# VITA-Group/UVC

Measured on AMD Instinct MI355X. Metric: images/sec UVC Stage-1 step, DeiT-Tiny budget=0.5, higher is better.
Workload: dtype bf16; 1 GPU; deit_tiny_patch16_224 Stage-1 UVC-train step, budget 0.5, per-GPU batch 512, 224x224x3 synthetic, soft distillation alpha 0.1, block gating on; global_batch=512, parallelism=dp1

## Files before the change

uvc_amd/csrc/fused_mlp.hip:

```cpp
#include "common.h"
#include "../../include/uvc_kernels.h"
#include <utility>
#include <algorithm>

namespace {

typedef bf16_t T;
constexpr int D = 192, KT = 6, RW = 2;
constexpr int W1S = D * 2 + 32;

__device__ __forceinline__ f32x4 mma(const bf16x8& a, const bf16x8& b, f32x4 c) {
  return __builtin_amdgcn_mfma_f32_16x16x32_bf16(a, b, c, 0, 0, 0);
}
__device__ __forceinline__ u32x4 pack8u(const f32x4& lo, const f32x4& hi) {
  u32x4 r;
  r[0] = pack_bf16x2(lo[0], lo[1]); r[1] = pack_bf16x2(lo[2], lo[3]);
  r[2] = pack_bf16x2(hi[0], hi[1]); r[3] = pack_bf16x2(hi[2], hi[3]);
  return r;
}
__device__ __forceinline__ bf16x8 pack8(const f32x4& lo, const f32x4& hi) { return __builtin_bit_cast(bf16x8, pack8u(lo, hi)); }

constexpr int V3_NW = 4, V3_NTH = 64 * V3_NW, V3_ROWS = V3_NW * RW * 16, V3_FC = 32;
constexpr int V3_W2S = V3_FC * 2 + 32;
constexpr int V3_W1B = V3_FC * W1S, V3_W2B = D * V3_W2S;
// ... 170 lines not shown
  f32x4 acc[RW][2], gpv[RW][2];
  auto fc1 = [&](int c) {
    const unsigned w1a = w1lane + (unsigned)((c & 1) * V3_BUF);
    const unsigned ba = b1lane + (unsigned)(c * (V3_FC * 4));
    u32x4 bi[2], f1[3][2];
    bi[0] = ds_rd<0>(ba); bi[1] = ds_rd<16>(ba);
    f1[0][0] = ds_rd<0>(w1a); f1[0][1] = ds_rd<16 * W1S>(w1a);
    f1[1][0] = ds_rd<64>(w1a); f1[1][1] = ds_rd<16 * W1S + 64>(w1a);
    __builtin_amdgcn_sched_barrier(0);
    static_for<KT>([&](auto ksv) {
      constexpr int ks = ksv.value, cur = ks % 3, nxt = (ks + 2) % 3;
      wait_tie2<(ks + 1 < KT) ? 2 : 0>(f1[cur][0], f1[cur][1]);
      if constexpr (ks == 0) asm volatile("" : "+v"(bi[0]), "+v"(bi[1]));
      static_for<2>([&](auto tv) {
        constexpr int t = tv.value;
        const bf16x8 af = __builtin_bit_cast(bf16x8, f1[cur][t]);
#pragma unroll
        for (int r = 0; r < RW; ++r) acc[r][t] = mma(af, hf[r][ks], ks == 0 ? __builtin_bit_cast(f32x4, bi[t]) : acc[r][t]);
        if constexpr (ks + 2 < KT) f1[nxt][t] = ds_rd<t * 16 * W1S + (ks + 2 < KT ? ks + 2 : 0) * 64>(w1a);
        __builtin_amdgcn_sched_barrier(0);
      });
    });
  };
  auto fc2_gelu = [&](auto fc2v, auto geluv, int cprev) {
    constexpr bool FC2 = decltype(fc2v)::value, GELU = decltype(geluv)::value;
    const unsigned w2a = w2lane + (unsigned)((cprev & 1) * V3_BUF);
    u32x4 f2[6];
    if constexpr (FC2) {
      static_for<6>([&](auto jv) { f2[jv.value] = ds_rd<jv.value * 16 * V3_W2S>(w2a); });
      __builtin_amdgcn_sched_barrier(0);
    }
    static_for<12>([&](auto jv) {
      constexpr int j = jv.value, slot = j % 6;
      if constexpr (FC2) {
        constexpr int younger = (j < 6) ? 5 : 11 - j;
        asm volatile("s_waitcnt lgkmcnt(%1)" : "+v"(f2[slot]) : "n"(younger));
        const bf16x8 af = __builtin_bit_cast(bf16x8, f2[slot]);
#pragma unroll
        for (int r = 0; r < RW; ++r) out[r][j] = mma(af, uf[r], out[r][j]);
        if constexpr (j + 6 < 12) f2[slot] = ds_rd<(j + 6 < 12 ? j + 6 : 0) * 16 * V3_W2S>(w2a);
      }
      if constexpr (GELU && j < 8) {
        constexpr int r = j >> 2, t = (j >> 1) & 1, e0 = (j & 1) * 2;
        if constexpr (TRAIN) {
          float f0, g0, f1, g1;
          Gelu<T>::fg(acc[r][t][e0], f0, g0);
          Gelu<T>::fg(acc[r][t][e0 + 1], f1, g1);
          acc[r][t][e0] = f0; gpv[r][t][e0] = g0; acc[r][t][e0 + 1] = f1; gpv[r][t][e0 + 1] = g1;
        } else {
          acc[r][t][e0] = Gelu<T>::f(acc[r][t][e0]);
          acc[r][t][e0 + 1] = Gelu<T>::f(acc[r][t][e0 + 1]);
        }
      }
      __builtin_amdgcn_sched_barrier(0);
    });
    if constexpr (GELU) {
#pragma unroll
      for (int r = 0; r < RW; ++r) {
        uf[r] = pack8(acc[r][0], acc[r][1]);
        if constexpr (TRAIN) {
          const int row = m0 + r * 16 + li;
          if (row < a.M) {
            const size_t o = (size_t)row * a.F + (size_t)(cprev + 1) * V3_FC + g * 8;
            *reinterpret_cast<u32x4*>(reinterpret_cast<T*>(a.u) + o) = __builtin_bit_cast(u32x4, uf[r]);
            *reinterpret_cast<u32x4*>(reinterpret_cast<T*>(a.gp) + o) = pack8u(gpv[r][0], gpv[r][1]);
          }
        }
      }
    }
  };
  auto end_iter = [&]() {
    asm volatile("s_waitcnt vmcnt(0)" ::: "memory");
    __builtin_amdgcn_s_barrier();
    __builtin_amdgcn_sched_barrier(0);
  };
  {
    dma(1, 0);
    __builtin_amdgcn_sched_barrier(0);
    fc1(0);
    fc2_gelu(std::false_type{}, std::true_type{}, -1);
    end_iter();
  }
  for (int c = 1; c < nch; ++c) {
    dma(c + 1, c);
    __builtin_amdgcn_sched_barrier(0);
    fc1(c);
    fc2_gelu(std::true_type{}, std::true_type{}, c - 1);
    end_iter();
  }
  fc2_gelu(std::true_type{}, std::false_type{}, nch - 1);

#pragma unroll
  for (int r = 0; r < RW; ++r) {
    const int row = m0 + r * 16 + li;
    if (row < a.M) {
      char* orow = reinterpret_cast<char*>(a.out) + (size_t)row * D * RSZ;
#pragma unroll
      for (int j = 0; j < D / 16; ++j) {
        const int col = j * 16 + g * 4;
        f32x4 o = out[r][j];
        if (a.gate) {
          f32x4 xp;
          if constexpr (RLOW) {
            const u32x2 q = *reinterpret_cast<const u32x2*>(reinterpret_cast<const bf16_t*>(a.x_prev) + (size_t)row * D + col);
            xp = f32x4{__uint_as_float(q[0] << 16), __uint_as_float(q[0] & 0xffff0000u), __uint_as_float(q[1] << 16), __uint_as_float(q[1] & 0xffff0000u)};
          } else xp = *reinterpret_cast<const f32x4*>(reinterpret_cast<const float*>(a.x_prev) + (size_t)row * D + col);
#pragma unroll
          for (int e = 0; e < 4; ++e) o[e] = __builtin_fmaf(d1, o[e], __builtin_fmaf(d0, xp[e], 0.0f));
        }
        if constexpr (RLOW) {
          u32x2 q; q[0] = pack_bf16x2(o[0], o[1]); q[1] = pack_bf16x2(o[2], o[3]);
          *reinterpret_cast<u32x2*>(orow + col * 2) = q;
          o = f32x4{__uint_as_float(q[0] << 16), __uint_as_float(q[0] & 0xffff0000u), __uint_as_float(q[1] << 16), __uint_as_float(q[1] & 0xffff0000u)};
        } else *reinterpret_cast<f32x4*>(orow + col * 4) = o;
        out[r][j] = o;
      }
    }
  }
  if (a.next_h) {
#pragma unroll
    for (int r = 0; r < RW; ++r) {
      const int row = m0 + r * 16 + li;
      float s = 0.f;
#pragma unroll
      for (int j = 0; j < D / 16; ++j) s += (out[r][j][0] + out[r][j][1]) + (out[r][j][2] + out[r][j][3]);
      s = sum_rows4(s);
      const float mean = s * (1.0f / D);
      float q = 0.f;
#pragma unroll
      for (int j = 0; j < D / 16; ++j)
#pragma unroll
        for (int e = 0; e < 4; ++e) { const float dd = out[r][j][e] - mean; q += dd * dd; }
      q = sum_rows4(q);
      const float rstd = rsqrtf(q * (1.0f / D) + a.eps);
      if (row < a.M) {
        if (a.next_mean && g == 0) { a.next_mean[row] = mean; a.next_rstd[row] = rstd; }
        T* hrow = reinterpret_cast<T*>(a.next_h) + (size_t)row * D;
#pragma unroll
        for (int j = 0; j < D / 16; ++j) {
          const int col = j * 16 + g * 4;
          const f32x4 gm = *reinterpret_cast<const f32x4*>(a.next_gamma + col), bt = *reinterpret_cast<const f32x4*>(a.next_beta + col);
          float y[4];
#pragma unroll
          for (int e = 0; e < 4; ++e) y[e] = (out[r][j][e] - mean) * rstd * gm[e] + bt[e];
          u32x2 pk; pk[0] = pack_bf16x2(y[0], y[1]); pk[1] = pack_bf16x2(y[2], y[3]);
          *reinterpret_cast<u32x2*>(hrow + col) = pk;
        }
      }
    }
  }
  asm volatile("s_waitcnt vmcnt(0)" ::: "memory");
}

constexpr int P_NW = 8, P_NTH = 64 * P_NW, P_MIN_ROWS = 16384, P_PASS = 13;
constexpr int P_W1B = V3_FC * D * 2, P_W2B = D * V3_FC * 2;
constexpr int P_BUF = P_W1B + P_W2B, P_NBUF = 3;
constexpr int P_XT = 16 * D * 2;
constexpr int P_OFF_X = P_NBUF * P_BUF;
constexpr int P_OFF_B1 = P_OFF_X + P_PASS * P_XT;
constexpr int P_OFF_GB = P_OFF_B1 + 4096, P_LDS = P_OFF_GB + 5 * D * 4;
constexpr int P_ND = (P_BUF / 1024 - P_NW / 2) / (P_NW / 2);
constexpr int P_NR = P_XT / 1024;
static_assert(P_LDS <= 160 * 1024, "one workgroup per CU");
static_assert(P_XT % 1024 == 0 && P_BUF == (P_ND + 1) * (P_NW / 2) * 1024 && P_PASS <= 13, "whole DMA instructions; four loader waves, four slots each");
static_assert(P_NW * P_XT + 256 < 65536, "second-tile offsets are ds_read immediates");

template <int OFF> __device__ __forceinline__ u32x2 ds_rd64(unsigned addr) {
  u32x2 v;
  asm volatile("ds_read_b64 %0, %1 offset:%2" : "=v"(v) : "v"(addr), "n"(OFF));
  return v;
}
__device__ __forceinline__ f32x4 bf4(const u32x2& q) {
  return f32x4{__uint_as_float(q[0] << 16), __uint_as_float(q[0] & 0xffff0000u), __uint_as_float(q[1] << 16), __uint_as_float(q[1] & 0xffff0000u)};
}
template <int N> __device__ __forceinline__ void wait_vm() { asm volatile("s_waitcnt vmcnt(%0)" ::"n"(N) : "memory"); }

__global__ __launch_bounds__(P_NTH, 1) void k_mlp_fused_p(uvc_mlp_args a, int ntiles) {
  extern __shared__ __attribute__((aligned(16))) char smem[];
  const int tid = threadIdx.x, lane = tid & 63, g = lane >> 4, li = lane & 15;
  const int w = __builtin_amdgcn_readfirstlane(tid >> 6);
  const int nch = a.F / V3_FC;
  {
    float* const sB1 = reinterpret_cast<float*>(smem + P_OFF_B1);
    float* const sG = reinterpret_cast<float*>(smem + P_OFF_GB);
    for (int i = tid; i < a.F; i += P_NTH) sB1[i] = a.b1[i];
    if (tid < D) {
      sG[tid] = a.gamma[tid]; sG[D + tid] = a.beta[tid]; sG[2 * D + tid] = a.b2[tid];
      if (a.next_h) { sG[3 * D + tid] = a.next_gamma[tid]; sG[4 * D + tid] = a.next_beta[tid]; }
    }
  }
  float d0 = 0.f, d1 = 1.f;
  if (a.gate) { d0 = a.gate[0]; d1 = a.gate[1]; }
  const unsigned s0 = lds_addr(smem);
  const int t0 = (int)((long long)blockIdx.x * ntiles / gridDim.x), t1 = (int)((long long)(blockIdx.x + 1) * ntiles / gridDim.x);
  int npass = (t1 - t0 + P_PASS - 1) / P_PASS;
  auto tile_rows = [&](int pb, int cnt, int k) { return (k < cnt) ? (pb + k) * 16 : a.M; };

  auto rowdma = [&](int npb, int ncnt, int q) {
    int ln = lane;
    asm volatile("" : "+v"(ln));
    const char* xb = reinterpret_cast<const char*>(a.x);
    const int slot = (q < 3 || w == P_NW / 2) ? (w & 3) + 4 * q : (w & 3) + 8;
    const int mb = tile_rows(npb, ncnt, slot);
#pragma unroll
    for (int i = 0; i < P_XT / 1024; ++i) {
      const int n = i * 64 + ln, row = n / 24, sp = n - row * 24;
      int grow = mb + row;
      grow = grow < a.M ? grow : a.M - 1;
      const unsigned off = (unsigned)grow * (unsigned)(D * 2) + (unsigned)((sp ^ ((row >> 1) & 7)) * 16);
      __builtin_amdgcn_global_load_lds((const void __attribute__((address_space(1)))*)(xb + (unsigned long long)off),
                                       (void __attribute__((address_space(3)))*)(smem + P_OFF_X + slot * P_XT + i * 1024), 16, 0, 0);
    }
  };

  unsigned doff[P_ND];
  const char* gsrc[P_ND];
  unsigned gstep[P_ND], ldst[P_ND];
  bool isw1[P_ND];
#pragma unroll
  for (int q = 0; q < P_ND; ++q) {
    const int j = (w < P_NW / 2) ? w : w + 4 * q;
    if (j < P_W1B / 1024) {
      const int n = j * 64 + lane, lr = n / 24, sp = n - lr * 24;
      const int h = ((lr >> 2) & 3) * 8 + (lr >> 4) * 4 + (lr & 3);
      doff[q] = (unsigned)(h * D * 2 + (sp ^ ((lr >> 1) & 7)) * 16);
      gsrc[q] = reinterpret_cast<const char*>(a.w1); gstep[q] = (unsigned)(V3_FC * D * 2);
      ldst[q] = (unsigned)(j * 1024);
    } else {
      const int jj = j - P_W1B / 1024;
      const int n = jj * 64 + lane, row = n >> 2, sp = n & 3;
      doff[q] = (unsigned)(row * a.F * 2 + (sp ^ ((4 - (row >> 2)) & 3)) * 16);
      gsrc[q] = reinterpret_cast<const char*>(a.w2); gstep[q] = (unsigned)(V3_FC * 2);
      ldst[q] = (unsigned)(P_W1B + jj * 1024);
    }
    isw1[q] = j < P_W1B / 1024;
  }
  auto dma = [&](auto nv, int c1, unsigned o1, int c2, unsigned o2) {
#pragma unroll
    for (int q = 0; q < decltype(nv)::value; ++q) {
      const int cc = isw1[q] ? c1 : c2;
      const char* src = gsrc[q] + (unsigned long long)((unsigned)cc * gstep[q] + doff[q]);
      char* dst = smem + ldst[q] + (isw1[q] ? o1 : o2);
      __builtin_amdgcn_global_load_lds((const void __attribute__((address_space(1)))*)src, (void __attribute__((address_space(3)))*)dst, 16, 0, 0);
    }
  };

  const int fx = (li >> 1) & 7;
  const unsigned sw0 = (unsigned)(li * (D * 2) + (g ^ fx) * 16), sw1 = (unsigned)(li * (D * 2) + ((4 + g) ^ fx) * 16);
  const unsigned xe0 = s0 + (unsigned)(P_OFF_X + w * P_XT) + sw0, xe1 = s0 + (unsigned)(P_OFF_X + w * P_XT) + sw1;
  unsigned xo[4];
#pragma unroll
  for (int q = 0; q < 4; ++q) xo[q] = s0 + (unsigned)(P_OFF_X + w * P_XT + li * (D * 2) + (((2 * q + (g >> 1)) ^ fx) * 16) + (g & 1) * 8);
  const unsigned w1e0 = s0 + sw0, w1e1 = s0 + sw1;
  const unsigned w2lane = s0 + (unsigned)(P_W1B + li * (V3_FC * 2) + ((g ^ ((4 - (li >> 2)) & 3)) * 16));
  const unsigned b1lane = s0 + (unsigned)(P_OFF_B1 + g * 32);
  const unsigned ga = s0 + (unsigned)(P_OFF_GB + g * 32), ba = ga + (unsigned)(D * 4);
  const unsigned b2a = s0 + (unsigned)(P_OFF_GB + 2 * D * 4 + g * 16), nga = b2a + (unsigned)(D * 4), nba = nga + (unsigned)(D * 4);

  unsigned o_cur = 0, o_nxt = P_BUF, o_nn = 2 * P_BUF;
  int pb = t0, cnt = (t1 - t0 + npass - 1) / (npass > 0 ? npass : 1);
  int mb0 = tile_rows(pb, cnt, w), mb1 = tile_rows(pb, cnt, P_NW + w);
  const bool loader = w >= P_NW / 2;
  if (loader) {
#pragma unroll
    for (int q = 0; q < 4; ++q) rowdma(pb, cnt, q);
    dma(std::integral_constant<int, P_ND>{}, 0, o_cur, 0, o_cur);
    dma(std::integral_constant<int, P_ND>{}, 1, o_nxt, 0, o_cur);
  } else {
    dma(std::integral_constant<int, 1>{}, 0, o_cur, 0, o_cur);
    dma(std::integral_constant<int, 1>{}, 1, o_nxt, 0, o_cur);
  }
  wait_vm<0>();
  __syncthreads();
  __builtin_amdgcn_sched_barrier(0);

  bf16x8 hf[RW][KT];
  f32x4 out[RW][D / 16];
  bf16x8 uf[RW];
  f32x4 acc[RW][2];

  auto pass = [&](auto ntv, auto ldv, int npb, int ncnt) {
    constexpr int NT = decltype(ntv)::value;
    constexpr bool LD = decltype(ldv)::value;
    static_for<NT>([&](auto rv) {
      constexpr int r = rv.value, XR = r * P_NW * P_XT;
      const int mb = r ? mb1 : mb0;
      u32x4 xq[KT];
      static_for<KT>([&](auto ksv) { constexpr int ks = ksv.value; xq[ks] = ds_rd<XR + (ks >> 1) * 128>((ks & 1) ? xe1 : xe0); });
      asm volatile("s_waitcnt lgkmcnt(0)" : "+v"(xq[0]), "+v"(xq[1]), "+v"(xq[2]), "+v"(xq[3]), "+v"(xq[4]), "+v"(xq[5]));
      f32x4 xv[2 * KT];
#pragma unroll
      for (int ks = 0; ks < KT; ++ks) {
        const u32x4 q = xq[ks];
        xv[2 * ks] = f32x4{__uint_as_float(q[0] << 16), __uint_as_float(q[0] & 0xffff0000u), __uint_as_float(q[1] << 16), __uint_as_float(q[1] & 0xffff0000u)};
        xv[2 * ks + 1] = f32x4{__uint_as_float(q[2] << 16), __uint_as_float(q[2] & 0xffff0000u), __uint_as_float(q[3] << 16), __uint_as_float(q[3] & 0xffff0000u)};
      }
      const float okf = (mb + li) < a.M ? 1.0f : 0.0f;
      float s = 0.f;
#pragma unroll
      for (int i = 0; i < 2 * KT; ++i) s += (xv[i][0] + xv[i][1]) + (xv[i][2] + xv[i][3]);
      s = sum_rows4(s);
      const float mean = s * (1.0f / D);
      float q = 0.f;
#pragma unroll
      for (int i = 0; i < 2 * KT; ++i)
#pragma unroll
        for (int e = 0; e < 4; ++e) { const float d = xv[i][e] - mean; q += d * d; }
      q = sum_rows4(q);
      const float rstd = rsqrtf(q * (1.0f / D) + a.eps);
      __builtin_amdgcn_sched_barrier(0);
      static_for<KT>([&](auto ksv) {
        constexpr int ks = ksv.value;
        u32x4 gq0 = ds_rd<ks * 128>(ga), gq1 = ds_rd<ks * 128 + 16>(ga), bq0 = ds_rd<ks * 128>(ba), bq1 = ds_rd<ks * 128 + 16>(ba);
        asm volatile("s_waitcnt lgkmcnt(0)" : "+v"(gq0), "+v"(gq1), "+v"(bq0), "+v"(bq1));
        const f32x4 g0 = __builtin_bit_cast(f32x4, gq0), g1 = __builtin_bit_cast(f32x4, gq1);
        const f32x4 b0 = __builtin_bit_cast(f32x4, bq0), b1 = __builtin_bit_cast(f32x4, bq1);
        f32x4 y0, y1;
#pragma unroll
        for (int e = 0; e < 4; ++e) {
          y0[e] = ((xv[2 * ks][e] - mean) * rstd * g0[e] + b0[e]) * okf;
          y1[e] = ((xv[2 * ks + 1][e] - mean) * rstd * g1[e] + b1[e]) * okf;
        }
        hf[r][ks] = pack8(y0, y1);
        asm volatile("" : "+v"(hf[r][ks]));
        __builtin_amdgcn_sched_barrier(0);
      });
      static_for<D / 64>([&](auto jqv) {
        constexpr int j0 = jqv.value * 4;
        u32x2 xr[4];
        u32x4 bq[4];
        static_for<4>([&](auto qv) {
          constexpr int j = j0 + qv.value;
          xr[qv.value] = ds_rd64<XR + (j >> 2) * 128>(xo[j & 3]);
          bq[qv.value] = ds_rd<j * 64>(b2a);
        });
        asm volatile("s_waitcnt lgkmcnt(0)" : "+v"(xr[0]), "+v"(xr[1]), "+v"(xr[2]), "+v"(xr[3]), "+v"(bq[0]), "+v"(bq[1]), "+v"(bq[2]), "+v"(bq[3]));
#pragma unroll
        for (int q4 = 0; q4 < 4; ++q4) {
          const f32x4 x4 = bf4(xr[q4]), bv = __builtin_bit_cast(f32x4, bq[q4]);
#pragma unroll
          for (int e = 0; e < 4; ++e) out[r][j0 + q4][e] = x4[e] + bv[e];
          asm volatile("" : "+v"(out[r][j0 + q4]));
        }
        __builtin_amdgcn_sched_barrier(0);
      });
    });
    __builtin_amdgcn_sched_barrier(0);

    auto fc1 = [&](int c) {
      const unsigned a0 = w1e0 + o_cur, a1 = w1e1 + o_cur;
      const unsigned bia = b1lane + (unsigned)(c * (V3_FC * 4));
      u32x4 bi[2], f1[3][2];
      bi[0] = ds_rd<0>(bia); bi[1] = ds_rd<16>(bia);
      f1[0][0] = ds_rd<0>(a0); f1[0][1] = ds_rd<16 * D * 2>(a0);
      f1[1][0] = ds_rd<0>(a1); f1[1][1] = ds_rd<16 * D * 2>(a1);
      __builtin_amdgcn_sched_barrier(0);
      static_for<KT>([&](auto ksv) {
        constexpr int ks = ksv.value, cur = ks % 3, nxt = (ks + 2) % 3;
        wait_tie2<(ks + 1 < KT) ? 2 : 0>(f1[cur][0], f1[cur][1]);
        if constexpr (ks == 0) asm volatile("" : "+v"(bi[0]), "+v"(bi[1]));
        static_for<2>([&](auto tv) {
          constexpr int t = tv.value;
          const bf16x8 af = __builtin_bit_cast(bf16x8, f1[cur][t]);
#pragma unroll
          for (int r = 0; r < NT; ++r) acc[r][t] = mma(af, hf[r][ks], ks == 0 ? __builtin_bit_cast(f32x4, bi[t]) : acc[r][t]);
          if constexpr (ks + 2 < KT) f1[nxt][t] = ds_rd<t * 16 * D * 2 + ((ks + 2 < KT ? ks + 2 : 0) >> 1) * 128>((ks & 1) ? a1 : a0);
          __builtin_amdgcn_sched_barrier(0);
        });
      });
    };
    auto fc2_gelu = [&](auto fc2v, auto geluv) {
      constexpr bool FC2 = decltype(fc2v)::value, GELU = decltype(geluv)::value;
      const unsigned w2a = w2lane + o_nn;
      u32x4 f2[6];
      if constexpr (FC2) {
        static_for<6>([&](auto jv) { f2[jv.value] = ds_rd<jv.value * 1024>(w2a); });
        __builtin_amdgcn_sched_barrier(0);
      }
      static_for<12>([&](auto jv) {
        constexpr int j = jv.value, slot = j % 6;
        if constexpr (FC2) {
          constexpr int younger = (j < 6) ? 5 : 11 - j;
          asm volatile("s_waitcnt lgkmcnt(%1)" : "+v"(f2[slot]) : "n"(younger));
          const bf16x8 af = __builtin_bit_cast(bf16x8, f2[slot]);
#pragma unroll
          for (int r = 0; r < NT; ++r) out[r][j] = mma(af, uf[r], out[r][j]);
          if constexpr (j + 6 < 12) f2[slot] = ds_rd<(j + 6 < 12 ? j + 6 : 0) * 1024>(w2a);
        }
        if constexpr (GELU && j < 8) {
          if constexpr (NT == 2) {
            constexpr int r = j >> 2, t = (j >> 1) & 1, e0 = (j & 1) * 2;
            acc[r][t][e0] = Gelu<T>::f(acc[r][t][e0]);
            acc[r][t][e0 + 1] = Gelu<T>::f(acc[r][t][e0 + 1]);
          } else {
            constexpr int t = j >> 2, e = j & 3;
            acc[0][t][e] = Gelu<T>::f(acc[0][t][e]);
          }
        }
        __builtin_amdgcn_sched_barrier(0);
      });
      if constexpr (GELU) {
#pragma unroll
        for (int r = 0; r < NT; ++r) uf[r] = pack8(acc[r][0], acc[r][1]);
      }
    };
    auto rotate = [&]() { const unsigned t = o_cur; o_cur = o_nxt; o_nxt = o_nn; o_nn = t; };
    auto request = [&](int c) {
      const int c1 = c + 2 < nch ? c + 2 : c + 2 - nch, c2 = c + 1 < nch ? c + 1 : 0;
      dma(std::integral_constant<int, LD ? P_ND : 1>{}, c1, o_nn, c2, o_nxt);
    };
    __builtin_amdgcn_s_barrier();
    __builtin_amdgcn_sched_barrier(0);
    {
      request(0);
      if constexpr (LD) rowdma(npb, ncnt, 0);
      __builtin_amdgcn_sched_barrier(0);
      fc1(0);
      fc2_gelu(std::false_type{}, std::true_type{});
      wait_vm<LD ? P_ND + P_NR : 1>();
      __builtin_amdgcn_s_barrier();
      __builtin_amdgcn_sched_barrier(0);
      rotate();
    }
#pragma nounroll
    for (int c = 1; c < 4; ++c) {
      request(c);
      if constexpr (LD) rowdma(npb, ncnt, c);
      __builtin_amdgcn_sched_barrier(0);
      fc1(c);
      fc2_gelu(std::true_type{}, std::true_type{});
      wait_vm<LD ? P_ND + 2 * P_NR : 1>();
      __builtin_amdgcn_s_barrier();
      __builtin_amdgcn_sched_barrier(0);
      rotate();
    }
#pragma nounroll
    for (int c = 4; c < nch; ++c) {
      request(c);
      __builtin_amdgcn_sched_barrier(0);
      fc1(c);
      fc2_gelu(std::true_type{}, std::true_type{});
      if (LD && c == 4) wait_vm<LD ? P_ND + P_NR : 1>(); else wait_vm<LD ? P_ND : 1>();
      __builtin_amdgcn_s_barrier();
      __builtin_amdgcn_sched_barrier(0);
      rotate();
    }
    fc2_gelu(std::true_type{}, std::false_type{});

    static_for<NT>([&](auto rv) {
      constexpr int r = rv.value;
      const int row = (r ? mb1 : mb0) + li;
      const bool ok = row < a.M;
      char* orow = reinterpret_cast<char*>(a.out) + (size_t)(ok ? row : 0) * (D * 2) + ((g & 1) * 16 + (g >> 1) * 8) * 2;
#pragma unroll
      for (int j = 0; j < D / 16; j += 2) {
        u32x2 q[2];
#pragma unroll
        for (int t = 0; t < 2; ++t) {
          f32x4 o = out[r][j + t];
          if (a.gate) {
            const f32x4 xp = bf4(*reinterpret_cast<const u32x2*>(reinterpret_cast<const bf16_t*>(a.x_prev) + (size_t)(ok ? row : 0) * D + (j + t) * 16 + g * 4));
#pragma unroll
            for (int e = 0; e < 4; ++e) o[e] = __builtin_fmaf(d1, o[e], __builtin_fmaf(d0, xp[e], 0.0f));
          }
          q[t][0] = pack_bf16x2(o[0], o[1]); q[t][1] = pack_bf16x2(o[2], o[3]);
          out[r][j + t] = bf4(q[t]);
        }
        const auto s0_ = __builtin_amdgcn_permlane16_swap(q[0][0], q[1][0], false, false);
        const auto s1_ = __builtin_amdgcn_permlane16_swap(q[0][1], q[1][1], false, false);
        if (ok) *reinterpret_cast<u32x4*>(orow + j * 32) = u32x4{s0_[0], s1_[0], s0_[1], s1_[1]};
      }
      if (a.next_h) {
        float s = 0.f;
#pragma unroll
        for (int j = 0; j < D / 16; ++j) s += (out[r][j][0] + out[r][j][1]) + (out[r][j][2] + out[r][j][3]);
        s = sum_rows4(s);
        const float mean = s * (1.0f / D);
        float q = 0.f;
#pragma unroll
        for (int j = 0; j < D / 16; ++j)
#pragma unroll
          for (int e = 0; e < 4; ++e) { const float dd = out[r][j][e] - mean; q += dd * dd; }
        q = sum_rows4(q);
        const float rstd = rsqrtf(q * (1.0f / D) + a.eps);
        if (ok && a.next_mean && g == 0) { a.next_mean[row] = mean; a.next_rstd[row] = rstd; }
        char* hrow = reinterpret_cast<char*>(a.next_h) + (size_t)(ok ? row : 0) * (D * 2) + ((g & 1) * 16 + (g >> 1) * 8) * 2;
        static_for<D / 64>([&](auto jqv) {
          constexpr int j0 = jqv.value * 4;
          u32x4 gq[4], bq[4];
          static_for<4>([&](auto qv) { gq[qv.value] = ds_rd<(j0 + qv.value) * 64>(nga); bq[qv.value] = ds_rd<(j0 + qv.value) * 64>(nba); });
          asm volatile("s_waitcnt lgkmcnt(0)" : "+v"(gq[0]), "+v"(gq[1]), "+v"(gq[2]), "+v"(gq[3]), "+v"(bq[0]), "+v"(bq[1]), "+v"(bq[2]), "+v"(bq[3]));
          u32x2 pk[4];
#pragma unroll
          for (int q4 = 0; q4 < 4; ++q4) {
            const f32x4 gm = __builtin_bit_cast(f32x4, gq[q4]), bt = __builtin_bit_cast(f32x4, bq[q4]);
            float y[4];
#pragma unroll
            for (int e = 0; e < 4; ++e) y[e] = (out[r][j0 + q4][e] - mean) * rstd * gm[e] + bt[e];
            pk[q4][0] = pack_bf16x2(y[0], y[1]); pk[q4][1] = pack_bf16x2(y[2], y[3]);
          }
#pragma unroll
          for (int q4 = 0; q4 < 4; q4 += 2) {
            const auto s0_ = __builtin_amdgcn_permlane16_swap(pk[q4][0], pk[q4 + 1][0], false, false);
            const auto s1_ = __builtin_amdgcn_permlane16_swap(pk[q4][1], pk[q4 + 1][1], false, false);
            if (ok) *reinterpret_cast<u32x4*>(hrow + (j0 + q4) * 32) = u32x4{s0_[0], s1_[0], s0_[1], s1_[1]};
          }
        });
      }
    });
    __builtin_amdgcn_sched_barrier(0);
  };

  for (int p = 0; p < npass; ++p) {
    const int npb = pb + cnt, left = npass - 1 - p;
    const int ncnt = left > 0 ? (t1 - npb + left - 1) / left : 0;
    if (loader) {
      if (mb1 < a.M) pass(std::integral_constant<int, 2>{}, std::true_type{}, npb, ncnt);
      else pass(std::integral_constant<int, 1>{}, std::true_type{}, npb, ncnt);
    } else {
      if (mb1 < a.M) pass(std::integral_constant<int, 2>{}, std::false_type{}, npb, ncnt);
      else pass(std::integral_constant<int, 1>{}, std::false_type{}, npb, ncnt);
    }
    pb = npb; cnt = ncnt;
    mb0 = tile_rows(pb, cnt, w); mb1 = tile_rows(pb, cnt, P_NW + w);
  }
  wait_vm<0>();
}

}

extern "C" int uvc_mlp_fused_supported(int32_t D_, int32_t F, int32_t dtype) { return D_ == D && F > 0 && F % 64 == 0 && F <= 1024 && dtype == UVC_BF16; }

extern "C" int uvc_mlp_fused_fwd(const uvc_mlp_args* p, void* stream) {
  if (!p || !p->x || !p->out || !p->gamma || !p->beta || !p->w1 || !p->b1 || !p->w2 || !p->b2) return uvc_set_error_msg(UVC_ERR_ARG, "uvc_mlp_fused_fwd: null pointer");
  if (p->M <= 0) return uvc_set_error_msg(UVC_ERR_ARG, "uvc_mlp_fused_fwd: empty");
  if (!uvc_mlp_fused_supported(p->D, p->F, UVC_BF16)) return uvc_set_error_msg(UVC_ERR_UNSUPPORTED, "uvc_mlp_fused_fwd: needs D == 192, F % 64 == 0 and F <= 1024");
  if ((((uintptr_t)p->x | (uintptr_t)p->out | (uintptr_t)p->w1 | (uintptr_t)p->w2 | (uintptr_t)p->b1 | (uintptr_t)p->x_prev | (uintptr_t)p->h |
        (uintptr_t)p->u | (uintptr_t)p->gp) & 15) != 0)
    return uvc_set_error_msg(UVC_ERR_ARG, "uvc_mlp_fused_fwd: buffers must be 16-byte aligned");
  const bool train = p->h || p->u || p->gp || p->mean || p->rstd;
  if (train && (!p->h || !p->u || !p->gp || !p->mean || !p->rstd)) return uvc_set_error_msg(UVC_ERR_ARG, "uvc_mlp_fused_fwd: training needs h, mean, rstd, gp and u");
  if ((p->gate != nullptr) != (p->x_prev != nullptr)) return uvc_set_error_msg(UVC_ERR_ARG, "uvc_mlp_fused_fwd: gate and x_prev come together");
  if (p->next_h && (!p->next_gamma || !p->next_beta || (((uintptr_t)p->next_h | (uintptr_t)p->next_gamma | (uintptr_t)p->next_beta) & 15) != 0))
    return uvc_set_error_msg(UVC_ERR_ARG, "uvc_mlp_fused_fwd: next_h needs 16-byte aligned next_gamma, next_beta");
  if ((p->next_mean != nullptr) != (p->next_rstd != nullptr) || (p->next_mean && !p->next_h))
    return uvc_set_error_msg(UVC_ERR_ARG, "uvc_mlp_fused_fwd: next_mean and next_rstd come together, with next_h");
  hipStream_t st = (hipStream_t)stream;
  {
#define MLP_ONE(TR_, RL_) { UVC_MAX_LDS(V3_LDS, k_mlp_fused_v3<TR_, RL_>); k_mlp_fused_v3<TR_, RL_><<<ceil_div(p->M, V3_ROWS), V3_NTH, V3_LDS, st>>>(*p); }
    if (p->rows_lowp && !train && p->M >= P_MIN_ROWS && p->F >= 256) {
      const int ntiles = ceil_div(p->M, 16);
      UVC_MAX_LDS(P_LDS, k_mlp_fused_p);
      k_mlp_fused_p<<<std::min(256, ceil_div(ntiles, P_PASS)), P_NTH, P_LDS, st>>>(*p, ntiles);
    } else if (p->rows_lowp) { if (train) MLP_ONE(true, true) else MLP_ONE(false, true) }
    else { if (train) MLP_ONE(true, false) else MLP_ONE(false, false) }
#undef MLP_ONE
    UVC_CHECK_LAUNCH();
    return UVC_OK;
  }
}
```

Measured before the change: 47450 images/sec.

## Restructure persistent fused MLP kernel to four waves with three tiles each

Replaces the 8-wave persistent fused MLP kernel, which split waves into loaders and compute waves, with a 4-wave version. Every wave now issues its share of weight and row DMA, interleaved into the fc1 k-steps, and handles up to three 16-row tiles. The fc1 of one chunk is software-pipelined with the fc2 of the previous chunk, with GELU spread across MFMA slots through sched_group_barrier. The goal is to hide LDS and DMA latency and keep more MFMA work in flight per wave. The cost is higher register pressure, and only one wave per SIMD means little latency hiding from occupancy. The path runs only for inference-mode calls with many rows (M >= 16384, not train), so its effect on a training-step benchmark is uncertain.

```diff
diff --git a/uvc_amd/csrc/fused_mlp.hip b/uvc_amd/csrc/fused_mlp.hip
--- a/uvc_amd/csrc/fused_mlp.hip
+++ b/uvc_amd/csrc/fused_mlp.hip
@@ -346,18 +346,18 @@
   asm volatile("s_waitcnt vmcnt(0)" ::: "memory");
 }
 
-constexpr int P_NW = 8, P_NTH = 64 * P_NW, P_MIN_ROWS = 16384, P_PASS = 13;
+constexpr int P_NW = 4, P_NTH = 64 * P_NW, P_MIN_ROWS = 16384, P_MAXNT = 3, P_PASS = P_NW * P_MAXNT;
 constexpr int P_W1B = V3_FC * D * 2, P_W2B = D * V3_FC * 2;
 constexpr int P_BUF = P_W1B + P_W2B, P_NBUF = 3;
 constexpr int P_XT = 16 * D * 2;
 constexpr int P_OFF_X = P_NBUF * P_BUF;
 constexpr int P_OFF_B1 = P_OFF_X + P_PASS * P_XT;
 constexpr int P_OFF_GB = P_OFF_B1 + 4096, P_LDS = P_OFF_GB + 5 * D * 4;
-constexpr int P_ND = (P_BUF / 1024 - P_NW / 2) / (P_NW / 2);
+constexpr int P_ND = P_BUF / 1024 / P_NW;
 constexpr int P_NR = P_XT / 1024;
 static_assert(P_LDS <= 160 * 1024, "one workgroup per CU");
-static_assert(P_XT % 1024 == 0 && P_BUF == (P_ND + 1) * (P_NW / 2) * 1024 && P_PASS <= 13, "whole DMA instructions; four loader waves, four slots each");
-static_assert(P_NW * P_XT + 256 < 65536, "second-tile offsets are ds_read immediates");
+static_assert(P_ND == KT && P_NR == KT && P_W1B == P_W2B && P_W1B / 1024 == P_NW * P_ND / 2, "one weight and one row instruction per fc1 k-step");
+static_assert(P_PASS == P_NW * P_MAXNT, "rows of iteration q < P_MAXNT: slot w + 4q");
 
 template <int OFF> __device__ __forceinline__ u32x2 ds_rd64(unsigned addr) {
   u32x2 v;
@@ -368,8 +368,21 @@
   return f32x4{__uint_as_float(q[0] << 16), __uint_as_float(q[0] & 0xffff0000u), __uint_as_float(q[1] << 16), __uint_as_float(q[1] & 0xffff0000u)};
 }
 template <int N> __device__ __forceinline__ void wait_vm() { asm volatile("s_waitcnt vmcnt(%0)" ::"n"(N) : "memory"); }
-
-__global__ __launch_bounds__(P_NTH, 1) void k_mlp_fused_p(uvc_mlp_args a, int ntiles) {
+template <int NT, int K> __device__ __forceinline__ void interleave() {
+#pragma unroll
+  for (int i = 0; i < NT; ++i) {
+    __builtin_amdgcn_sched_group_barrier(0x008, 1, 0);
+    __builtin_amdgcn_sched_group_barrier(0x002, K, 0);
+  }
+}
+template <int U, int NT> __device__ __forceinline__ void gelu_unit(f32x4 (&h)[NT]) {
+  static_for<4 * NT>([&](auto vv) {
+    constexpr int v = vv.value;
+    if constexpr (v * 12 / (4 * NT) == U) h[v >> 2][v & 3] = Gelu<T>::f(h[v >> 2][v & 3]);
+  });
+}
+
+__global__ __launch_bounds__(P_NTH, 1) __attribute__((amdgpu_waves_per_eu(1, 1))) void k_mlp_fused_p4(uvc_mlp_args a, int ntiles) {
   extern __shared__ __attribute__((aligned(16))) char smem[];
   const int tid = threadIdx.x, lane = tid & 63, g = lane >> 4, li = lane & 15;
   const int w = __builtin_amdgcn_readfirstlane(tid >> 6);
@@ -387,64 +400,47 @@
   if (a.gate) { d0 = a.gate[0]; d1 = a.gate[1]; }
   const unsigned s0 = lds_addr(smem);
   const int t0 = (int)((long long)blockIdx.x * ntiles / gridDim.x), t1 = (int)((long long)(blockIdx.x + 1) * ntiles / gridDim.x);
-  int npass = (t1 - t0 + P_PASS - 1) / P_PASS;
+  const int npass = (t1 - t0 + P_PASS - 1) / P_PASS;
   auto tile_rows = [&](int pb, int cnt, int k) { return (k < cnt) ? (pb + k) * 16 : a.M; };
 
-  auto rowdma = [&](int npb, int ncnt, int q) {
+  auto rowdma = [&](int npb, int ncnt, int q, int i) {
     int ln = lane;
     asm volatile("" : "+v"(ln));
     const char* xb = reinterpret_cast<const char*>(a.x);
-    const int slot = (q < 3 || w == P_NW / 2) ? (w & 3) + 4 * q : (w & 3) + 8;
+    const int slot = w + P_NW * q;
     const int mb = tile_rows(npb, ncnt, slot);
-#pragma unroll
-    for (int i = 0; i < P_XT / 1024; ++i) {
-      const int n = i * 64 + ln, row = n / 24, sp = n - row * 24;
-      int grow = mb + row;
-      grow = grow < a.M ? grow : a.M - 1;
-      const unsigned off = (unsigned)grow * (unsigned)(D * 2) + (unsigned)((sp ^ ((row >> 1) & 7)) * 16);
-      __builtin_amdgcn_global_load_lds((const void __attribute__((address_space(1)))*)(xb + (unsigned long long)off),
-                                       (void __attribute__((address_space(3)))*)(smem + P_OFF_X + slot * P_XT + i * 1024), 16, 0, 0);
-    }
+    const int n = i * 64 + ln, row = n / 24, sp = n - row * 24;
+    int grow = mb + row;
+    grow = grow < a.M ? grow : a.M - 1;
+    const unsigned off = (unsigned)grow * (unsigned)(D * 2) + (unsigned)((sp ^ ((row >> 1) & 7)) * 16);
+    __builtin_amdgcn_global_load_lds((const void __attribute__((address_space(1)))*)(xb + (unsigned long long)off),
+                                     (void __attribute__((address_space(3)))*)(smem + P_OFF_X + slot * P_XT + i * 1024), 16, 0, 0);
   };
 
   unsigned doff[P_ND];
-  const char* gsrc[P_ND];
-  unsigned gstep[P_ND], ldst[P_ND];
-  bool isw1[P_ND];
 #pragma unroll
   for (int q = 0; q < P_ND; ++q) {
-    const int j = (w < P_NW / 2) ? w : w + 4 * q;
-    if (j < P_W1B / 1024) {
+    const int j = w + P_NW * (q % 3);
+    if (q < 3) {
       const int n = j * 64 + lane, lr = n / 24, sp = n - lr * 24;
       const int h = ((lr >> 2) & 3) * 8 + (lr >> 4) * 4 + (lr & 3);
       doff[q] = (unsigned)(h * D * 2 + (sp ^ ((lr >> 1) & 7)) * 16);
-      gsrc[q] = reinterpret_cast<const char*>(a.w1); gstep[q] = (unsigned)(V3_FC * D * 2);
-      ldst[q] = (unsigned)(j * 1024);
     } else {
-      const int jj = j - P_W1B / 1024;
-      const int n = jj * 64 + lane, row = n >> 2, sp = n & 3;
+      const int n = j * 64 + lane, row = n >> 2, sp = n & 3;
       doff[q] = (unsigned)(row * a.F * 2 + (sp ^ ((4 - (row >> 2)) & 3)) * 16);
-      gsrc[q] = reinterpret_cast<const char*>(a.w2); gstep[q] = (unsigned)(V3_FC * 2);
-      ldst[q] = (unsigned)(P_W1B + jj * 1024);
-    }
-    isw1[q] = j < P_W1B / 1024;
-  }
-  auto dma = [&](auto nv, int c1, unsigned o1, int c2, unsigned o2) {
-#pragma unroll
-    for (int q = 0; q < decltype(nv)::value; ++q) {
-      const int cc = isw1[q] ? c1 : c2;
-      const char* src = gsrc[q] + (unsigned long long)((unsigned)cc * gstep[q] + doff[q]);
-      char* dst = smem + ldst[q] + (isw1[q] ? o1 : o2);
-      __builtin_amdgcn_global_load_lds((const void __attribute__((address_space(1)))*)src, (void __attribute__((address_space(3)))*)dst, 16, 0, 0);
-    }
+    }
+  }
+  auto dma = [&](auto qv, int c1, unsigned o1, int c2, unsigned o2) {
+    constexpr int q = decltype(qv)::value;
+    constexpr bool W1 = q < 3;
+    const int j = w + P_NW * (q % 3);
+    const char* src = reinterpret_cast<const char*>(W1 ? a.w1 : a.w2) + (unsigned long long)((unsigned)(W1 ? c1 : c2) * (unsigned)(W1 ? V3_FC * D * 2 : V3_FC * 2) + doff[q]);
+    char* dst = smem + (W1 ? 0 : P_W1B) + j * 1024 + (W1 ? o1 : o2);
+    __builtin_amdgcn_global_load_lds((const void __attribute__((address_space(1)))*)src, (void __attribute__((address_space(3)))*)dst, 16, 0, 0);
   };
 
   const int fx = (li >> 1) & 7;
   const unsigned sw0 = (unsigned)(li * (D * 2) + (g ^ fx) * 16), sw1 = (unsigned)(li * (D * 2) + ((4 + g) ^ fx) * 16);
-  const unsigned xe0 = s0 + (unsigned)(P_OFF_X + w * P_XT) + sw0, xe1 = s0 + (unsigned)(P_OFF_X + w * P_XT) + sw1;
-  unsigned xo[4];
-#pragma unroll
-  for (int q = 0; q < 4; ++q) xo[q] = s0 + (unsigned)(P_OFF_X + w * P_XT + li * (D * 2) + (((2 * q + (g >> 1)) ^ fx) * 16) + (g & 1) * 8);
   const unsigned w1e0 = s0 + sw0, w1e1 = s0 + sw1;
   const unsigned w2lane = s0 + (unsigned)(P_W1B + li * (V3_FC * 2) + ((g ^ ((4 - (li >> 2)) & 3)) * 16));
   const unsigned b1lane = s0 + (unsigned)(P_OFF_B1 + g * 32);
@@ -453,34 +449,29 @@
 
   unsigned o_cur = 0, o_nxt = P_BUF, o_nn = 2 * P_BUF;
   int pb = t0, cnt = (t1 - t0 + npass - 1) / (npass > 0 ? npass : 1);
-  int mb0 = tile_rows(pb, cnt, w), mb1 = tile_rows(pb, cnt, P_NW + w);
-  const bool loader = w >= P_NW / 2;
-  if (loader) {
-#pragma unroll
-    for (int q = 0; q < 4; ++q) rowdma(pb, cnt, q);
-    dma(std::integral_constant<int, P_ND>{}, 0, o_cur, 0, o_cur);
-    dma(std::integral_constant<int, P_ND>{}, 1, o_nxt, 0, o_cur);
-  } else {
-    dma(std::integral_constant<int, 1>{}, 0, o_cur, 0, o_cur);
-    dma(std::integral_constant<int, 1>{}, 1, o_nxt, 0, o_cur);
-  }
+#pragma unroll
+  for (int q = 0; q < P_MAXNT; ++q)
+#pragma unroll
+    for (int i = 0; i < P_NR; ++i) rowdma(pb, cnt, q, i);
+  static_for<P_ND>([&](auto qv) { dma(qv, 0, o_cur, 0, o_cur); });
+  static_for<3>([&](auto qv) { dma(qv, 1, o_nxt, 0, o_cur); });
   wait_vm<0>();
   __syncthreads();
   __builtin_amdgcn_sched_barrier(0);
 
-  bf16x8 hf[RW][KT];
-  f32x4 out[RW][D / 16];
-  bf16x8 uf[RW];
-  f32x4 acc[RW][2];
-
-  auto pass = [&](auto ntv, auto ldv, int npb, int ncnt) {
+  auto pass = [&](auto ntv, int npb, int ncnt) {
     constexpr int NT = decltype(ntv)::value;
-    constexpr bool LD = decltype(ldv)::value;
+    int mb[NT];
+#pragma unroll
+    for (int r = 0; r < NT; ++r) mb[r] = tile_rows(pb, cnt, w + P_NW * r);
+    bf16x8 hf[NT][KT];
+    f32x4 out[NT][D / 16];
     static_for<NT>([&](auto rv) {
-      constexpr int r = rv.value, XR = r * P_NW * P_XT;
-      const int mb = r ? mb1 : mb0;
+      constexpr int r = rv.value;
+      const unsigned xt = s0 + (unsigned)(P_OFF_X + (w + P_NW * r) * P_XT);
+      const unsigned xe0 = xt + sw0, xe1 = xt + sw1;
       u32x4 xq[KT];
-      static_for<KT>([&](auto ksv) { constexpr int ks = ksv.value; xq[ks] = ds_rd<XR + (ks >> 1) * 128>((ks & 1) ? xe1 : xe0); });
+      static_for<KT>([&](auto ksv) { constexpr int ks = ksv.value; xq[ks] = ds_rd<(ks >> 1) * 128>((ks & 1) ? xe1 : xe0); });
       asm volatile("s_waitcnt lgkmcnt(0)" : "+v"(xq[0]), "+v"(xq[1]), "+v"(xq[2]), "+v"(xq[3]), "+v"(xq[4]), "+v"(xq[5]));
       f32x4 xv[2 * KT];
 #pragma unroll
@@ -489,7 +480,7 @@
         xv[2 * ks] = f32x4{__uint_as_float(q[0] << 16), __uint_as_float(q[0] & 0xffff0000u), __uint_as_float(q[1] << 16), __uint_as_float(q[1] & 0xffff0000u)};
         xv[2 * ks + 1] = f32x4{__uint_as_float(q[2] << 16), __uint_as_float(q[2] & 0xffff0000u), __uint_as_float(q[3] << 16), __uint_as_float(q[3] & 0xffff0000u)};
       }
-      const float okf = (mb + li) < a.M ? 1.0f : 0.0f;
+      const float okf = (mb[r] + li) < a.M ? 1.0f : 0.0f;
       float s = 0.f;
 #pragma unroll
       for (int i = 0; i < 2 * KT; ++i) s += (xv[i][0] + xv[i][1]) + (xv[i][2] + xv[i][3]);
@@ -525,7 +516,8 @@
         u32x4 bq[4];
         static_for<4>([&](auto qv) {
           constexpr int j = j0 + qv.value;
-          xr[qv.value] = ds_rd64<XR + (j >> 2) * 128>(xo[j & 3]);
+          const unsigned xo = xt + (unsigned)(li * (D * 2) + (((2 * (j & 3) + (g >> 1)) ^ fx) * 16) + (g & 1) * 8);
+          xr[qv.value] = ds_rd64<(j >> 2) * 128>(xo);
           bq[qv.value] = ds_rd<j * 64>(b2a);
         });
         asm volatile("s_waitcnt lgkmcnt(0)" : "+v"(xr[0]), "+v"(xr[1]), "+v"(xr[2]), "+v"(xr[3]), "+v"(bq[0]), "+v"(bq[1]), "+v"(bq[2]), "+v"(bq[3]));
@@ -541,109 +533,109 @@
     });
     __builtin_amdgcn_sched_barrier(0);
 
-    auto fc1 = [&](int c) {
-      const unsigned a0 = w1e0 + o_cur, a1 = w1e1 + o_cur;
-      const unsigned bia = b1lane + (unsigned)(c * (V3_FC * 4));
-      u32x4 bi[2], f1[3][2];
-      bi[0] = ds_rd<0>(bia); bi[1] = ds_rd<16>(bia);
-      f1[0][0] = ds_rd<0>(a0); f1[0][1] = ds_rd<16 * D * 2>(a0);
-      f1[1][0] = ds_rd<0>(a1); f1[1][1] = ds_rd<16 * D * 2>(a1);
-      __builtin_amdgcn_sched_barrier(0);
-      static_for<KT>([&](auto ksv) {
-        constexpr int ks = ksv.value, cur = ks % 3, nxt = (ks + 2) % 3;
-        wait_tie2<(ks + 1 < KT) ? 2 : 0>(f1[cur][0], f1[cur][1]);
-        if constexpr (ks == 0) asm volatile("" : "+v"(bi[0]), "+v"(bi[1]));
-        static_for<2>([&](auto tv) {
-          constexpr int t = tv.value;
-          const bf16x8 af = __builtin_bit_cast(bf16x8, f1[cur][t]);
-#pragma unroll
-          for (int r = 0; r < NT; ++r) acc[r][t] = mma(af, hf[r][ks], ks == 0 ? __builtin_bit_cast(f32x4, bi[t]) : acc[r][t]);
-          if constexpr (ks + 2 < KT) f1[nxt][t] = ds_rd<t * 16 * D * 2 + ((ks + 2 < KT ? ks + 2 : 0) >> 1) * 128>((ks & 1) ? a1 : a0);
-          __builtin_amdgcn_sched_barrier(0);
-        });
-      });
-    };
-    auto fc2_gelu = [&](auto fc2v, auto geluv) {
-      constexpr bool FC2 = decltype(fc2v)::value, GELU = decltype(geluv)::value;
+    f32x4 accA[NT], accB[NT], pend[NT];
+    u32x2 ufl[NT];
+    bf16x8 uf[NT];
+    auto iter = [&](auto fc1v, auto fc2v, auto rowsv, int c) {
+      constexpr bool FC1 = decltype(fc1v)::value, FC2 = decltype(fc2v)::value, ROWS = decltype(rowsv)::value;
+      constexpr bool GB = FC2, GA = FC1;
       const unsigned w2a = w2lane + o_nn;
       u32x4 f2[6];
+      if constexpr (FC1) {
+        const int c1 = c + 2 < nch ? c + 2 : c + 2 - nch, c2 = c + 1 < nch ? c + 1 : 0;
+        const unsigned a0 = w1e0 + o_cur, a1 = w1e1 + o_cur;
+        const unsigned bia = b1lane + (unsigned)(c * (V3_FC * 4));
+        u32x4 bi[2], f1[3][2];
+        bi[0] = ds_rd<0>(bia); bi[1] = ds_rd<16>(bia);
+        f1[0][0] = ds_rd<0>(a0); f1[0][1] = ds_rd<16 * D * 2>(a0);
+        f1[1][0] = ds_rd<0>(a1); f1[1][1] = ds_rd<16 * D * 2>(a1);
+        __builtin_amdgcn_sched_barrier(0);
+        static_for<KT>([&](auto ksv) {
+          constexpr int ks = ksv.value, cur = ks % 3, nxt = (ks + 2) % 3;
+          wait_tie2<(ks + 1 < KT) ? 2 : (FC2 ? 3 : 0)>(f1[cur][0], f1[cur][1]);
+          if constexpr (ks == 0) asm volatile("" : "+v"(bi[0]), "+v"(bi[1]));
+          static_for<2>([&](auto tv) {
+            constexpr int t = tv.value, u = ks * 2 + t;
+            const bf16x8 af = __builtin_bit_cast(bf16x8, f1[cur][t]);
+            f32x4 (&acc)[NT] = t ? accB : accA;
+#pragma unroll
+            for (int r = 0; r < NT; ++r) acc[r] = mma(af, hf[r][ks], ks == 0 ? __builtin_bit_cast(f32x4, bi[t]) : acc[r]);
+            if constexpr (ks + 2 < KT) f1[nxt][t] = ds_rd<t * 16 * D * 2 + ((ks + 2 < KT ? ks + 2 : 0) >> 1) * 128>((ks & 1) ? a1 : a0);
+            if constexpr (FC2 && ks >= 4)
+              static_for<6>([&](auto iv) {
+                constexpr int i = iv.value;
+                if constexpr (8 + i * 4 / 6 == u) f2[i] = ds_rd<i * 1024>(w2a);
+              });
+            if constexpr (t == 0) dma(std::integral_constant<int, ks>{}, c1, o_nn, c2, o_nxt);
+            else if constexpr (ROWS) rowdma(npb, ncnt, c, ks);
+            if constexpr (GB) gelu_unit<u, NT>(pend);
+            interleave<NT, GB ? (NT >= 3 ? 3 : 5) : 2>();
+            __builtin_amdgcn_sched_barrier(0);
+          });
+        });
+      } else if constexpr (GB) {
+        static_for<12>([&](auto uv) { gelu_unit<uv.value, NT>(pend); });
+      }
+      if constexpr (GB) {
+#pragma unroll
+        for (int r = 0; r < NT; ++r) uf[r] = __builtin_bit_cast(bf16x8, u32x4{ufl[r][0], ufl[r][1], pack_bf16x2(pend[r][0], pend[r][1]), pack_bf16x2(pend[r][2], pend[r][3])});
+      }
+      __builtin_amdgcn_sched_barrier(0);
       if constexpr (FC2) {
-        static_for<6>([&](auto jv) { f2[jv.value] = ds_rd<jv.value * 1024>(w2a); });
-        __builtin_amdgcn_sched_barrier(0);
-      }
-      static_for<12>([&](auto jv) {
-        constexpr int j = jv.value, slot = j % 6;
-        if constexpr (FC2) {
+        if constexpr (!FC1) {
+          static_for<6>([&](auto iv) { f2[iv.value] = ds_rd<iv.value * 1024>(w2a); });
+          __builtin_amdgcn_sched_barrier(0);
+        }
+        static_for<12>([&](auto jv) {
+          constexpr int j = jv.value, slot = j % 6;
           constexpr int younger = (j < 6) ? 5 : 11 - j;
           asm volatile("s_waitcnt lgkmcnt(%1)" : "+v"(f2[slot]) : "n"(younger));
           const bf16x8 af = __builtin_bit_cast(bf16x8, f2[slot]);
 #pragma unroll
           for (int r = 0; r < NT; ++r) out[r][j] = mma(af, uf[r], out[r][j]);
           if constexpr (j + 6 < 12) f2[slot] = ds_rd<(j + 6 < 12 ? j + 6 : 0) * 1024>(w2a);
-        }
-        if constexpr (GELU && j < 8) {
-          if constexpr (NT == 2) {
-            constexpr int r = j >> 2, t = (j >> 1) & 1, e0 = (j & 1) * 2;
-            acc[r][t][e0] = Gelu<T>::f(acc[r][t][e0]);
-            acc[r][t][e0 + 1] = Gelu<T>::f(acc[r][t][e0 + 1]);
-          } else {
-            constexpr int t = j >> 2, e = j & 3;
-            acc[0][t][e] = Gelu<T>::f(acc[0][t][e]);
-          }
-        }
-        __builtin_amdgcn_sched_barrier(0);
-      });
-      if constexpr (GELU) {
-#pragma unroll
-        for (int r = 0; r < NT; ++r) uf[r] = pack8(acc[r][0], acc[r][1]);
-      }
+          if constexpr (GA) gelu_unit<j, NT>(accA);
+          interleave<NT, GA ? (NT >= 3 ? 3 : 5) : 1>();
+          __builtin_amdgcn_sched_barrier(0);
+        });
+      } else if constexpr (GA) {
+        static_for<12>([&](auto uv) { gelu_unit<uv.value, NT>(accA); });
+      }
+      if constexpr (GA) {
+#pragma unroll
+        for (int r = 0; r < NT; ++r) {
+          ufl[r] = u32x2{pack_bf16x2(accA[r][0], accA[r][1]), pack_bf16x2(accA[r][2], accA[r][3])};
+          pend[r] = accB[r];
+        }
+      }
+      __builtin_amdgcn_sched_barrier(0);
     };
     auto rotate = [&]() { const unsigned t = o_cur; o_cur = o_nxt; o_nxt = o_nn; o_nn = t; };
-    auto request = [&](int c) {
-      const int c1 = c + 2 < nch ? c + 2 : c + 2 - nch, c2 = c + 1 < nch ? c + 1 : 0;
-      dma(std::integral_constant<int, LD ? P_ND : 1>{}, c1, o_nn, c2, o_nxt);
+    auto end_iter = [&](auto rowsv) {
+      wait_vm<decltype(rowsv)::value ? P_ND + P_NR : P_ND>();
+      __builtin_amdgcn_s_barrier();
+      __builtin_amdgcn_sched_barrier(0);
+      rotate();
     };
     __builtin_amdgcn_s_barrier();
     __builtin_amdgcn_sched_barrier(0);
-    {
-      request(0);
-      if constexpr (LD) rowdma(npb, ncnt, 0);
-      __builtin_amdgcn_sched_barrier(0);
-      fc1(0);
-      fc2_gelu(std::false_type{}, std::true_type{});
-      wait_vm<LD ? P_ND + P_NR : 1>();
-      __builtin_amdgcn_s_barrier();
-      __builtin_amdgcn_sched_barrier(0);
-      rotate();
-    }
+    iter(std::true_type{}, std::false_type{}, std::true_type{}, 0);
+    end_iter(std::true_type{});
 #pragma nounroll
-    for (int c = 1; c < 4; ++c) {
-      request(c);
-      if constexpr (LD) rowdma(npb, ncnt, c);
-      __builtin_amdgcn_sched_barrier(0);
-      fc1(c);
-      fc2_gelu(std::true_type{}, std::true_type{});
-      wait_vm<LD ? P_ND + 2 * P_NR : 1>();
-      __builtin_amdgcn_s_barrier();
-      __builtin_amdgcn_sched_barrier(0);
-      rotate();
+    for (int c = 1; c < P_MAXNT; ++c) {
+      iter(std::true_type{}, std::true_type{}, std::true_type{}, c);
+      end_iter(std::true_type{});
     }
 #pragma nounroll
-    for (int c = 4; c < nch; ++c) {
-      request(c);
-      __builtin_amdgcn_sched_barrier(0);
-      fc1(c);
-      fc2_gelu(std::true_type{}, std::true_type{});
-      if (LD && c == 4) wait_vm<LD ? P_ND + P_NR : 1>(); else wait_vm<LD ? P_ND : 1>();
-      __builtin_amdgcn_s_barrier();
-      __builtin_amdgcn_sched_barrier(0);
-      rotate();
-    }
-    fc2_gelu(std::true_type{}, std::false_type{});
+    for (int c = P_MAXNT; c < nch; ++c) {
+      iter(std::true_type{}, std::true_type{}, std::false_type{}, c);
+      end_iter(std::false_type{});
+    }
+    iter(std::false_type{}, std::true_type{}, std::false_type{}, nch);
 
     static_for<NT>([&](auto rv) {
       constexpr int r = rv.value;
-      const int row = (r ? mb1 : mb0) + li;
+      const int row = mb[r] + li;
       const bool ok = row < a.M;
       char* orow = reinterpret_cast<char*>(a.out) + (size_t)(ok ? row : 0) * (D * 2) + ((g & 1) * 16 + (g >> 1) * 8) * 2;
 #pragma unroll
@@ -708,15 +700,11 @@
   for (int p = 0; p < npass; ++p) {
     const int npb = pb + cnt, left = npass - 1 - p;
     const int ncnt = left > 0 ? (t1 - npb + left - 1) / left : 0;
-    if (loader) {
-      if (mb1 < a.M) pass(std::integral_constant<int, 2>{}, std::true_type{}, npb, ncnt);
-      else pass(std::integral_constant<int, 1>{}, std::true_type{}, npb, ncnt);
-    } else {
-      if (mb1 < a.M) pass(std::integral_constant<int, 2>{}, std::false_type{}, npb, ncnt);
-      else pass(std::integral_constant<int, 1>{}, std::false_type{}, npb, ncnt);
-    }
+    const int own = (cnt - w + P_NW - 1) / P_NW;
+    if (own >= 3) pass(std::integral_constant<int, 3>{}, npb, ncnt);
+    else if (own == 2) pass(std::integral_constant<int, 2>{}, npb, ncnt);
+    else pass(std::integral_constant<int, 1>{}, npb, ncnt);
     pb = npb; cnt = ncnt;
-    mb0 = tile_rows(pb, cnt, w); mb1 = tile_rows(pb, cnt, P_NW + w);
   }
   wait_vm<0>();
 }
@@ -744,8 +732,8 @@
 #define MLP_ONE(TR_, RL_) { UVC_MAX_LDS(V3_LDS, k_mlp_fused_v3<TR_, RL_>); k_mlp_fused_v3<TR_, RL_><<<ceil_div(p->M, V3_ROWS), V3_NTH, V3_LDS, st>>>(*p); }
     if (p->rows_lowp && !train && p->M >= P_MIN_ROWS && p->F >= 256) {
       const int ntiles = ceil_div(p->M, 16);
-      UVC_MAX_LDS(P_LDS, k_mlp_fused_p);
-      k_mlp_fused_p<<<std::min(256, ceil_div(ntiles, P_PASS)), P_NTH, P_LDS, st>>>(*p, ntiles);
+      UVC_MAX_LDS(P_LDS, k_mlp_fused_p4);
+      k_mlp_fused_p4<<<std::min(256, ceil_div(ntiles, P_PASS)), P_NTH, P_LDS, st>>>(*p, ntiles);
     } else if (p->rows_lowp) { if (train) MLP_ONE(true, true) else MLP_ONE(false, true) }
     else { if (train) MLP_ONE(true, false) else MLP_ONE(false, false) }
 #undef MLP_ONE
```

Result: slower. 46550 images/sec (median of 6 runs) (-1.9%).
